# microsoft/GenerativeImage2Text

Hardware: NVIDIA H100
Metric: captions/sec (greedy, max_len=40) GIT_BASE batch64 (higher is better)
Workload: dtype bf16

## Files before the change

### generativeimage2text_b200/csrc/gemm.cuh

```cuda
#pragma once
#include "ptx.cuh"

namespace gitb200 {

struct GemmParams {
  int M, N, K;
  int k_splits;
  int transposed;
  int partial;
  long long split_stride;
  int act;
  int out_bf16;
  const float* bias;
  const float* resid;
  long long ld_resid;
  void* out[3];
  long long ldo;
  long long batch_stride;
  int seg_n;
  int rows_per_batch;
  int row_offset;
  const int* skip;
  unsigned long long* dbg;
  int split3;
  int pdl;
  ChainSync chain;
  const int* lse_target;
};

constexpr int EPI_TRANSPOSED = 1, EPI_BF16 = 2, EPI_RESID = 4, EPI_PARTIAL = 8, EPI_ACT_SHIFT = 4, EPI_SPLIT3 = 64;
constexpr int EPI_LSE = 128;
constexpr int epi_code(bool transposed, bool bf16, bool resid, bool partial, int act) {
  return (transposed ? EPI_TRANSPOSED : 0) | (bf16 ? EPI_BF16 : 0) | (resid ? EPI_RESID : 0) | (partial ? EPI_PARTIAL : 0) |
         (act << EPI_ACT_SHIFT);
}

template <int ACT>
__device__ __forceinline__ float act_ct(float x) {
  return apply_act(x, ACT);
}

template <int BN>
struct GemmCfg {
  static constexpr int BM = 128;
  static constexpr int BK = 64;
  static constexpr int A_BYTES = BM * BK * 2;
  static constexpr int B_BYTES = BN * BK * 2;
  static constexpr int STAGE_BYTES = A_BYTES + B_BYTES;
  static constexpr int MMA_WGS = 2;
  static constexpr int THREADS = 128 * (1 + MMA_WGS);
  static constexpr int WG_STAGING_BYTES = 4 * 32 * 128;
  static constexpr int STAGING_BYTES = MMA_WGS * WG_STAGING_BYTES;
  static constexpr int BAR_BYTES = 256;
  static constexpr int SMEM_LIMIT = 227 * 1024;
  static constexpr int STAGES_RAW = (SMEM_LIMIT - 1024 - BAR_BYTES - STAGING_BYTES) / STAGE_BYTES;
  static constexpr int STAGES = STAGES_RAW > 8 ? 8 : STAGES_RAW;
  static constexpr int SMEM_BYTES = STAGES * STAGE_BYTES + STAGING_BYTES + 1024 + BAR_BYTES;
  static constexpr int PRODUCER_REGS = 40, MMA_REGS = 232;
  static_assert(BN % 64 == 0 && BN >= 64 && BN <= 256, "BN");
  static_assert(B_BYTES % 1024 == 0, "B tile must keep 1024B alignment for SWIZZLE_128B");
  static_assert(2 * STAGES * 8 <= BAR_BYTES, "barrier area");
  static_assert(STAGES >= 3, "pipeline depth");
};

__device__ __forceinline__ uint32_t epi_row_offsets(const GemmParams& p, int row0, int rsub, bool store_ok, long long (&ooff)[8]) {
  uint32_t okmask = 0;
  int bq = (row0 + rsub) / p.rows_per_batch;
  int sq = (row0 + rsub) - bq * p.rows_per_batch;
#pragma unroll
  for (int it = 0; it < 8; ++it) {
    if (row0 + it * 4 + rsub < p.M && store_ok) okmask |= 1u << it;
    ooff[it] = (static_cast<long long>(bq) * p.batch_stride + sq + p.row_offset) * p.ldo;
    sq += 4;
    while (sq >= p.rows_per_batch) { sq -= p.rows_per_batch; ++bq; }
  }
  return okmask;
}

template <int EPI>
__device__ __forceinline__ void epi_store_normal(const GemmParams& p, const uint8_t* stg, int lane, int n0,
                                                 int row0, const long long (&ooff)[8], uint32_t okmask) {
  constexpr bool kBf16 = (EPI & EPI_BF16) != 0;
  constexpr bool kResid = (EPI & EPI_RESID) != 0;
  constexpr int kAct = (EPI >> EPI_ACT_SHIFT) & 3;
  constexpr bool kSplit3 = (EPI & EPI_SPLIT3) != 0;
  static_assert(!kSplit3 || kBf16, "split3 is a bf16 output format");
  const int c4 = lane & 7;
  const int rsub = lane >> 3;
  float4 b4 = make_float4(0.f, 0.f, 0.f, 0.f);
  if (p.bias != nullptr) b4 = __ldg(reinterpret_cast<const float4*>(p.bias + n0) + c4);
  int seg = 0;
  if (p.seg_n < p.N) seg = n0 / p.seg_n;
  const int nn = n0 - seg * p.seg_n + c4 * 4;
  float4 v[8];
#pragma unroll
  for (int it = 0; it < 8; ++it) {
    const int rr = it * 4 + rsub;
    v[it] = *reinterpret_cast<const float4*>(stg + rr * 128 + ((c4 ^ (rr & 7)) << 4));
  }
  float4 res[8];
  if (kResid) {
    const float* rbase = p.resid + static_cast<long long>(row0 + rsub) * p.ld_resid + n0 + c4 * 4;
#pragma unroll
    for (int it = 0; it < 8; ++it) {
      res[it] = make_float4(0.f, 0.f, 0.f, 0.f);
      if (okmask & (1u << it)) res[it] = *reinterpret_cast<const float4*>(rbase + static_cast<long long>(it) * 4 * p.ld_resid);
    }
  }
  uint8_t* obase = reinterpret_cast<uint8_t*>(p.out[seg]) + static_cast<long long>(nn) * (kBf16 ? 2 : 4);
#pragma unroll
  for (int it = 0; it < 8; ++it) {
    float4 o = v[it];
    o.x += b4.x; o.y += b4.y; o.z += b4.z; o.w += b4.w;
    if (kAct != ACT_NONE) {
      o.x = act_ct<kAct>(o.x); o.y = act_ct<kAct>(o.y); o.z = act_ct<kAct>(o.z); o.w = act_ct<kAct>(o.w);
// ... 81 lines not shown
        }
      } else {
        float* dst = reinterpret_cast<float*>(p.out[0]) + off;
        if (full4 && (p.ldo & 3) == 0) {
          *reinterpret_cast<float4*>(dst) = make_float4(v[0], v[1], v[2], v[3]);
        } else if (full4 && (p.ldo & 1) == 0) {
          *reinterpret_cast<float2*>(dst) = make_float2(v[0], v[1]);
          *reinterpret_cast<float2*>(dst + 2) = make_float2(v[2], v[3]);
        } else {
          for (int e = 0; e < 4; ++e)
            if (f0 + e < p.M) dst[e] = v[e];
        }
      }
    }
  }
}

__device__ __forceinline__ void epi_lse_accum(const GemmParams& p, const uint8_t* stg, int lane, int n0, const int (&tgt)[8],
                                              float (&m)[8], float (&se)[8], float (&sx)[8], float (&xt)[8]) {
  const int c4 = lane & 7;
  const int rsub = lane >> 3;
  const int col0 = n0 + c4 * 4;
  float b[4];
  bool ok[4];
#pragma unroll
  for (int e = 0; e < 4; ++e) {
    ok[e] = col0 + e < p.N;
    b[e] = ok[e] ? __ldg(p.bias + col0 + e) : 0.f;
  }
#pragma unroll
  for (int it = 0; it < 8; ++it) {
    const int rr = it * 4 + rsub;
    const float4 v = *reinterpret_cast<const float4*>(stg + rr * 128 + ((c4 ^ (rr & 7)) << 4));
    const float x[4] = {v.x + b[0], v.y + b[1], v.z + b[2], v.w + b[3]};
    float cm = -INFINITY;
#pragma unroll
    for (int e = 0; e < 4; ++e) if (ok[e]) cm = fmaxf(cm, x[e]);
    const float nm = fmaxf(m[it], cm);
    if (nm == -INFINITY) continue;
    float acc = (m[it] == -INFINITY) ? 0.f : se[it] * __expf(m[it] - nm);
#pragma unroll
    for (int e = 0; e < 4; ++e) {
      if (ok[e]) {
        acc += __expf(x[e] - nm);
        sx[it] += x[e];
        if (tgt[it] == col0 + e) xt[it] = x[e];
      }
    }
    se[it] = acc;
    m[it] = nm;
  }
}

template <int BN, int EPI>
__global__ void __launch_bounds__(GemmCfg<BN>::THREADS, 1)
gemm_bf16_wgmma(const __grid_constant__ CUtensorMap tmA, const __grid_constant__ CUtensorMap tmB,
                const GemmParams p) {
  using C = GemmCfg<BN>;
  constexpr bool kTransposed = (EPI & EPI_TRANSPOSED) != 0;
  constexpr bool kLse = (EPI & EPI_LSE) != 0;
  static_assert(!kLse || EPI == EPI_LSE, "the statistics epilogue takes no other option");
  if (p.pdl) griddep_launch_early();
  if (p.pdl) tl_mark(100000 + 1000 + static_cast<int>(gridDim.x));
  if ((!p.pdl || p.chain.counters != nullptr) && p.skip != nullptr && *p.skip != 0) return;
  extern __shared__ __align__(1024) uint8_t smem_raw[];
  uint8_t* smem = smem_raw + ((1024u - (smem_u32(smem_raw) & 1023u)) & 1023u);
  uint8_t* sA = smem;
  uint8_t* sB = smem + C::STAGES * C::A_BYTES;
  uint8_t* sStage = smem + C::STAGES * C::STAGE_BYTES;
  uint64_t* full = reinterpret_cast<uint64_t*>(sStage + C::STAGING_BYTES);
  uint64_t* empty = full + C::STAGES;

  const int wg = threadIdx.x >> 7;
  const int warp = (threadIdx.x >> 5) & 3;
  const int lane = threadIdx.x & 31;

  if (threadIdx.x == 0) {
    tma_prefetch_desc(&tmA);
    tma_prefetch_desc(&tmB);
    for (int s = 0; s < C::STAGES; ++s) {
      mbar_init(&full[s], 1);
      mbar_init(&empty[s], C::MMA_WGS);
    }
    mbar_fence_init();
  }
  __syncthreads();

  const int m_tiles = (p.M + C::BM - 1) / C::BM;
  const int n_tiles = (p.N + BN - 1) / BN;
  const int kb_total = (p.K + C::BK - 1) / C::BK;
  const int kb_per = (kb_total + p.k_splits - 1) / p.k_splits;
  const int mn_tiles = m_tiles * n_tiles;
  const int num_tiles = mn_tiles * p.k_splits;

  const bool chained = p.chain.counters != nullptr;
  int npre = 0;
  if (kTransposed && p.pdl && static_cast<int>(blockIdx.x) < num_tiles) {
    const int split = static_cast<int>(blockIdx.x) / mn_tiles;
    const int kb0 = split * kb_per;
    npre = min(C::STAGES, min(kb_total, kb0 + kb_per) - kb0);
    if (threadIdx.x == 0) {
      const int m_blk = (static_cast<int>(blockIdx.x) - split * mn_tiles) / n_tiles;
      for (int i = 0; i < npre; ++i) {
        mbar_arrive_expect_tx(&full[i], C::STAGE_BYTES);
        tma_load_2d(sA + i * C::A_BYTES, &tmA, &full[i], (kb0 + i) * C::BK, m_blk * C::BM);
      }
    }
  }
  if (chained) chain_wait(p.chain);
  else if (p.pdl) griddep_wait();
  if (p.pdl) tl_mark(1000 + static_cast<int>(gridDim.x));

  if (wg == 0) {
    setmaxnreg_dec<C::PRODUCER_REGS>();
    if (threadIdx.x == 0) {
      int stage = 0;
      uint32_t phase = 0;
      for (int tile = blockIdx.x; tile < num_tiles; tile += gridDim.x) {
        const int split = tile / mn_tiles;
        const int rem = tile - split * mn_tiles;
        const int m_blk = rem / n_tiles;
        const int n_blk = rem - m_blk * n_tiles;
        const int kb0 = split * kb_per;
        const int kb1 = min(kb_total, kb0 + kb_per);
        for (int kb = kb0; kb < kb1; ++kb) {
          if (npre > 0) {
            --npre;
            tma_load_2d(sB + stage * C::B_BYTES, &tmB, &full[stage], kb * C::BK, n_blk * BN);
          } else {
            mbar_wait(&empty[stage], phase ^ 1);
            mbar_arrive_expect_tx(&full[stage], C::STAGE_BYTES);
            tma_load_2d(sA + stage * C::A_BYTES, &tmA, &full[stage], kb * C::BK, m_blk * C::BM);
            tma_load_2d(sB + stage * C::B_BYTES, &tmB, &full[stage], kb * C::BK, n_blk * BN);
          }
          if (++stage == C::STAGES) {
            stage = 0;
            phase ^= 1;
          }
        }
      }
    }
  } else {
    setmaxnreg_inc<C::MMA_REGS>();
    const int mw = wg - 1;
    const bool store_ok = !(p.pdl && !chained && p.skip != nullptr && *p.skip != 0);
    uint8_t* stg_wg = sStage + mw * C::WG_STAGING_BYTES;
    uint8_t* stg = stg_wg + warp * (32 * 128);
    const int rsub = lane >> 3;
    float acc[BN / 2];
    int stage = 0;
    uint32_t phase = 0;
    for (int tile = blockIdx.x; tile < num_tiles; tile += gridDim.x) {
      const int split = tile / mn_tiles;
      const int rem = tile - split * mn_tiles;
      const int m_blk = rem / n_tiles;
      const int n_blk = rem - m_blk * n_tiles;
      const int kb0 = split * kb_per;
      const int kb1 = min(kb_total, kb0 + kb_per);
      int prev = -1;
      for (int kb = kb0; kb < kb1; ++kb) {
        mbar_wait(&full[stage], phase);
        if (p.pdl && tile == static_cast<int>(blockIdx.x) && kb == kb0 && threadIdx.x == 128) tl_mark_one(300000 + 1000 + static_cast<int>(gridDim.x));
        const uint32_t a_base = smem_u32(sA + stage * C::A_BYTES + mw * (64 * 128));
        const uint32_t b_base = smem_u32(sB + stage * C::B_BYTES);
        wgmma_fence();
#pragma unroll
        for (int k = 0; k < C::BK / 16; ++k)
          Wgmma<BN>::mma(acc, wgmma_desc_sw128(a_base + k * 32), wgmma_desc_sw128(b_base + k * 32), (kb > kb0 || k > 0) ? 1u : 0u);
        wgmma_commit();
        if (prev >= 0) {
          wgmma_wait<1>();
          if ((threadIdx.x & 127) == 0) mbar_arrive(&empty[prev]);
        }
        prev = stage;
        if (++stage == C::STAGES) {
          stage = 0;
          phase ^= 1;
        }
      }
      wgmma_wait<0>();
      if ((threadIdx.x & 127) == 0) mbar_arrive(&empty[prev]);
      if (p.pdl && tile == static_cast<int>(blockIdx.x) && threadIdx.x == 128) tl_mark_one(400000 + 1000 + static_cast<int>(gridDim.x));

      const int row0 = m_blk * C::BM + mw * 64 + (warp & 1) * 32;
      long long ooff[8];
      uint32_t okmask = 0;
      if (!kTransposed && !kLse) okmask = epi_row_offsets(p, row0, rsub, store_ok, ooff);
      float lm[8], lse_s[8], lsx[8], lxt[8];
      int ltg[8];
      if constexpr (kLse) {
#pragma unroll
        for (int it = 0; it < 8; ++it) {
          const int row = row0 + it * 4 + rsub;
          ltg[it] = row < p.M ? p.lse_target[row] : -1;
          lm[it] = -INFINITY; lse_s[it] = 0.f; lsx[it] = 0.f; lxt[it] = 0.f;
        }
      }
#pragma unroll
      for (int cc = 0; cc < BN / 64; ++cc) {
        if (n_blk * BN + cc * 64 >= p.N) break;
#pragma unroll
        for (int j8 = 0; j8 < 8; ++j8) {
#pragma unroll
          for (int hh = 0; hh < 2; ++hh) {
            const int r64 = warp * 16 + (lane >> 2) + 8 * hh;
            const int c64 = j8 * 8 + 2 * (lane & 3);
            const int r = r64 & 31, c = c64 & 31;
            uint8_t* blk = stg_wg + ((c64 >> 5) * 2 + (r64 >> 5)) * (32 * 128);
            const float v0 = acc[4 * (cc * 8 + j8) + 2 * hh], v1 = acc[4 * (cc * 8 + j8) + 2 * hh + 1];
            if (!kTransposed) {
              *reinterpret_cast<float2*>(blk + r * 128 + (((c >> 2) ^ (r & 7)) << 4) + (c & 3) * 4) = make_float2(v0, v1);
            } else {
              *reinterpret_cast<float*>(blk + c * 128 + (((r >> 2) ^ (c & 7)) << 4) + (r & 3) * 4) = v0;
              *reinterpret_cast<float*>(blk + (c + 1) * 128 + (((r >> 2) ^ ((c + 1) & 7)) << 4) + (r & 3) * 4) = v1;
            }
          }
        }
        named_bar_sync(1 + mw, 128);
        const int n0 = n_blk * BN + cc * 64 + (warp >> 1) * 32;
        if constexpr (kLse) {
          epi_lse_accum(p, stg, lane, n0, ltg, lm, lse_s, lsx, lxt);
        } else if (!kTransposed) {
          if (n0 < p.N) epi_store_normal<EPI>(p, stg, lane, n0, row0, ooff, okmask);
        } else {
          epi_store_transposed<EPI>(p, stg, lane, n0, row0, split, store_ok);
        }
        named_bar_sync(1 + mw, 128);
      }
      if constexpr (kLse) {
#pragma unroll
        for (int it = 0; it < 8; ++it) {
#pragma unroll
          for (int o = 1; o < 8; o <<= 1) {
            const float m_o = __shfl_xor_sync(0xffffffffu, lm[it], o);
            const float s_o = __shfl_xor_sync(0xffffffffu, lse_s[it], o);
            const float nm = fmaxf(lm[it], m_o);
            const float sa = (lm[it] == -INFINITY) ? 0.f : lse_s[it] * __expf(lm[it] - nm);
            const float sb = (m_o == -INFINITY) ? 0.f : s_o * __expf(m_o - nm);
            lse_s[it] = sa + sb;
            lm[it] = nm;
            lsx[it] += __shfl_xor_sync(0xffffffffu, lsx[it], o);
            lxt[it] += __shfl_xor_sync(0xffffffffu, lxt[it], o);
          }
          const int row = row0 + it * 4 + rsub;
          if ((lane & 7) == 0 && row < p.M)
            reinterpret_cast<float4*>(p.out[0])[static_cast<long long>(row) * p.ldo + 2 * n_blk + (warp >> 1)] =
                make_float4(lm[it], lse_s[it], lsx[it], lxt[it]);
        }
      }
    }
  }

  __syncthreads();
  if (p.pdl) tl_mark(200000 + 1000 + static_cast<int>(gridDim.x));
  if (chained && threadIdx.x == 0) chain_signal_thread0(p.chain);
}

}
```

### generativeimage2text_b200/csrc/gitb200.cu

```cuda
#include <cuda.h>
#include <cuda_bf16.h>
#include <cuda_runtime.h>

#include <algorithm>
#include <cmath>
#include <cstdarg>
#include <cstdio>
#include <cstring>
#include <map>
#include <mutex>
#include <set>
#include <string>
#include <utility>
#include <vector>

#include "../../include/gitb200.h"
#include "attention.cuh"
#include "constrained.cuh"
#include "decode_mega.cuh"
#include "gemm.cuh"
#include "preproc.cuh"
#include "ptx.cuh"
#include "rowops.cuh"
#include "search.cuh"
// ... 1 lines not shown
using namespace gitb200;
typedef __nv_bfloat16 bf16;

#define GITB200_ABI_VERSION 10

static thread_local std::string g_create_error;

struct DevBuf {
  void* p = nullptr;
  size_t cap = 0;
  bool owned = true;
  cudaError_t ensure(size_t bytes) {
    if (bytes <= cap) return cudaSuccess;
    if (!owned) return cudaErrorInvalidValue;
    if (p) cudaFree(p);
    p = nullptr;
    cap = 0;
    cudaError_t e = cudaMalloc(&p, bytes);
    if (e == cudaSuccess) cap = bytes;
    return e;
  }
  void release() {
    if (p && owned) cudaFree(p);
    p = nullptr;
    cap = 0;
    owned = true;
  }
  void borrow(const DevBuf& o) {
    release();
    p = o.p;
    cap = o.cap;
    owned = false;
  }
  template <typename T>
  T* as() const { return reinterpret_cast<T*>(p); }
};

struct EncLayer {
  DevBuf wqkv, bqkv, wo, bo, ln1g, ln1b, ln2g, ln2b, w1, b1, w2, b2;
};
struct DecLayer {
  DevBuf wqkv, bqkv, wo, bo, lnag, lnab, w1, b1, w2, b2, lnog, lnob;
  DevBuf m_wqkv, m_wo, m_w1, m_w2;
};

typedef CUresult (*EncodeTiledFn)(CUtensorMap*, CUtensorMapDataType, cuuint32_t, void*, const cuuint64_t*,
                                  const cuuint64_t*, const cuuint32_t*, const cuuint32_t*, CUtensorMapInterleave,
                                  CUtensorMapSwizzle, CUtensorMapL2promotion, CUtensorMapFloatOOBfill);

struct TmapKey {
  const void* ptr;
  long long rows, cols, ld;
  int box_rows;
  bool operator<(const TmapKey& o) const {
    if (ptr != o.ptr) return ptr < o.ptr;
    if (rows != o.rows) return rows < o.rows;
    if (cols != o.cols) return cols < o.cols;
    if (ld != o.ld) return ld < o.ld;
    return box_rows < o.box_rows;
  }
};

struct DecAttnGeom {
  int chunk_rows, box_rows;
  size_t smem;
  int grid;
};

struct gitb200_engine {
  gitb200_config cfg;
  int device = 0;
  int num_sms = 132;
  std::string err;
  int64_t launches = 0;
  bool use_graph = true;
  bool use_pdl = true;
  bool use_mega = true;
  bool mega_ready = false;
  int debug_layers = -1;
  bool parity = false;
  int ks() const { return parity ? 3 : 1; }
  size_t kvb() const { return parity ? 4 : 2; }
  const gitb200_engine* weights_from = nullptr;

  int g = 0, L = 0, Kpatch = 0, Kp = 0, d = 0, D = 0, F = 0, V = 0;
  int in_h = 0, in_w = 0, gh = 0, gw = 0, Lc = 0;
  std::vector<int> rg_next_hw;
  bool cur_ragged = false;
  std::vector<int> cur_lens;
  DevBuf rg_tab, rg_lens;

  DevBuf w_patch, cls, pos_emb, lnpre_g, lnpre_b, lnpost_g, lnpost_b;
  std::vector<EncLayer> enc;
  DevBuf w_vp, b_vp, lnvp_g, lnvp_b, words_f32, words_bf16, positions, lnemb_g, lnemb_b, out_bias, temb;
  DevBuf m_lm;
  std::vector<DecLayer> dec;
  std::set<std::string> seen;
  bool finalized = false;

  DevBuf x, h, qkv, ctx, u, feats, feats_f32, pos_interp;
  DevBuf pt, pxd, phd, pq, pctx, pu;
  DevBuf img_kv, txt_kv, src_row[2];
  size_t txt_kv_eb = 0;
  DevBuf xd_t, hd_t, qkv_t, ctx_t, t_t, u_t, logits;
  DevBuf y_t, qb_t, mega_bar;
  DevBuf state, next_token, logprob_sum, tokens_i64, stage_img, stage_tok, stage_lp, prefix_dev;
  DevBuf beam_ws;
// ... 45 lines not shown
  va_list ap;
  va_start(ap, fmt);
  vsnprintf(buf, sizeof(buf), fmt, ap);
  va_end(ap);
  if (h) h->err = buf; else g_create_error = buf;
  return 1;
}

#define CK(call)                                                                                     \
  do {                                                                                               \
    cudaError_t e_ = (call);                                                                         \
    if (e_ != cudaSuccess) return fail(h, "%s failed: %s (%s:%d)", #call, cudaGetErrorString(e_), __FILE__, __LINE__); \
  } while (0)
#define CKL(h_, what)                                                                                \
  do {                                                                                               \
    cudaError_t e_ = cudaGetLastError();                                                             \
    if (e_ != cudaSuccess) return fail(h_, "launch %s failed: %s", what, cudaGetErrorString(e_));    \
    (h_)->launches++;                                                                                \
  } while (0)
#define TRY(expr)                 \
  do {                            \
    int rc_ = (expr);             \
    if (rc_ != 0) return rc_;     \
  } while (0)

template <typename... KArgs, typename... Args>
static cudaError_t launch_k(bool pdl, void (*kern)(KArgs...), dim3 grid, dim3 block, size_t smem, cudaStream_t st,
                            Args&&... args) {
  cudaLaunchConfig_t cfg{};
  cfg.gridDim = grid;
  cfg.blockDim = block;
  cfg.dynamicSmemBytes = smem;
  cfg.stream = st;
  cudaLaunchAttribute attr[1];
  attr[0].id = cudaLaunchAttributeProgrammaticStreamSerialization;
  attr[0].val.programmaticStreamSerializationAllowed = 1;
  cfg.attrs = attr;
  cfg.numAttrs = pdl ? 1 : 0;
  return cudaLaunchKernelEx(&cfg, kern, std::forward<Args>(args)...);
}

static int load_encode_fn(gitb200_engine* h) {
  if (h->encode_tiled) return 0;
  void* fn = nullptr;
  cudaDriverEntryPointQueryResult qres;
  cudaError_t e = cudaGetDriverEntryPoint("cuTensorMapEncodeTiled", &fn, cudaEnableDefault, &qres);
  if (e != cudaSuccess || qres != cudaDriverEntryPointSuccess || fn == nullptr)
    return fail(h, "cuTensorMapEncodeTiled not available from the driver: %s", cudaGetErrorString(e));
  h->encode_tiled = reinterpret_cast<EncodeTiledFn>(fn);
  return 0;
}

static int get_tmap(gitb200_engine* h, const void* ptr, long long rows, long long cols, long long ld, int box_rows,
                    CUtensorMap* out, bool swizzle = true) {
  TmapKey key{ptr, rows, cols, ld, swizzle ? box_rows : -box_rows};
  auto it = h->tmaps.find(key);
  if (it != h->tmaps.end()) {
    *out = it->second;
    return 0;
  }
  TRY(load_encode_fn(h));
  if ((reinterpret_cast<uintptr_t>(ptr) & 15) != 0 || (ld * 2) % 16 != 0)
    return fail(h, "TMA operand must be 16-byte aligned with a 16-byte multiple row pitch (ptr=%p ld=%lld)", ptr, ld);
  CUtensorMap m;
  cuuint64_t dims[2] = {static_cast<cuuint64_t>(cols), static_cast<cuuint64_t>(rows)};
  cuuint64_t strides[1] = {static_cast<cuuint64_t>(ld) * 2};
  cuuint32_t box[2] = {64u, static_cast<cuuint32_t>(box_rows)};
  cuuint32_t estr[2] = {1u, 1u};
  CUresult r = h->encode_tiled(&m, CU_TENSOR_MAP_DATA_TYPE_BFLOAT16, 2, const_cast<void*>(ptr), dims, strides, box, estr,
                               CU_TENSOR_MAP_INTERLEAVE_NONE, swizzle ? CU_TENSOR_MAP_SWIZZLE_128B : CU_TENSOR_MAP_SWIZZLE_NONE,
                               CU_TENSOR_MAP_L2_PROMOTION_L2_256B, CU_TENSOR_MAP_FLOAT_OOB_FILL_NONE);
  if (r != CUDA_SUCCESS) return fail(h, "cuTensorMapEncodeTiled failed with CUresult %d (rows=%lld cols=%lld ld=%lld box=%d)",
                                     static_cast<int>(r), rows, cols, ld, box_rows);
  if (h->tmaps.size() > 4096) h->tmaps.clear();
  h->tmaps[key] = m;
  *out = m;
  return 0;
}

struct GemmCall {
  const bf16* A = nullptr;
  long long lda = 0;
  const bf16* B = nullptr;
  long long ldb = 0;
  GemmParams p{};
  int bn = 0;
};

template <int BN, int EPI>
static int launch_gemm_inst(gitb200_engine* h, const GemmCall& c, cudaStream_t st) {
  using C = GemmCfg<BN>;
  static bool attr_set[64] = {false};
  if (!attr_set[h->device & 63]) {
    CK(cudaFuncSetAttribute(gemm_bf16_wgmma<BN, EPI>, cudaFuncAttributeMaxDynamicSharedMemorySize, C::SMEM_BYTES));
    attr_set[h->device & 63] = true;
  }
  CUtensorMap ta, tb;
  TRY(get_tmap(h, c.A, c.p.M, c.p.K, c.lda, 128, &ta));
  TRY(get_tmap(h, c.B, c.p.N, c.p.K, c.ldb, BN, &tb));
  const int m_tiles = (c.p.M + 127) / 128;
  const int n_tiles = (c.p.N + BN - 1) / BN;
  const int tiles = m_tiles * n_tiles * c.p.k_splits;
  const int grid = tiles < h->num_sms ? tiles : h->num_sms;
  h->last_gemm_grid = grid;
  CK(launch_k(c.p.pdl != 0, gemm_bf16_wgmma<BN, EPI>, dim3(grid), dim3(C::THREADS), C::SMEM_BYTES, st, ta, tb, c.p));
  CKL(h, "gemm_bf16_wgmma");
  return 0;
}

template <int BN>
static int launch_gemm_bn(gitb200_engine* h, const GemmCall& c, cudaStream_t st) {
  const GemmParams& p = c.p;
  if constexpr (BN == 256) {
    if (p.lse_target != nullptr) return launch_gemm_inst<BN, EPI_LSE>(h, c, st);
  }
  if (p.lse_target != nullptr) return fail(h, "gemm: the LM-head statistics epilogue runs with 256-column tiles only");
  const int code = epi_code(p.transposed != 0, p.out_bf16 != 0, p.resid != nullptr, p.partial != 0, p.act) | (p.split3 ? EPI_SPLIT3 : 0);
  if constexpr (BN == 256) {
    switch (code) {
      case epi_code(false, true, false, false, ACT_QUICKGELU_EXACT) | EPI_SPLIT3: return launch_gemm_inst<BN, epi_code(false, true, false, false, ACT_QUICKGELU_EXACT) | EPI_SPLIT3>(h, c, st);
      case epi_code(false, true, false, false, ACT_GELU_ERF) | EPI_SPLIT3: return launch_gemm_inst<BN, epi_code(false, true, false, false, ACT_GELU_ERF) | EPI_SPLIT3>(h, c, st);
      default: break;
    }
  }
  if constexpr (BN == 64 || BN == 128 || BN == 256) {
    if (code == (epi_code(true, true, false, false, ACT_GELU_ERF) | EPI_SPLIT3))
      return launch_gemm_inst<BN, epi_code(true, true, false, false, ACT_GELU_ERF) | EPI_SPLIT3>(h, c, st);
  }
  if constexpr (BN == 192 || BN == 256 || BN == 128) {
    switch (code) {
      case epi_code(false, true, false, false, ACT_NONE): return launch_gemm_inst<BN, epi_code(false, true, false, false, ACT_NONE)>(h, c, st);
      case epi_code(false, false, true, false, ACT_NONE): return launch_gemm_inst<BN, epi_code(false, false, true, false, ACT_NONE)>(h, c, st);
      case epi_code(false, false, false, false, ACT_NONE): return launch_gemm_inst<BN, epi_code(false, false, false, false, ACT_NONE)>(h, c, st);
      case epi_code(false, true, false, false, ACT_QUICKGELU): return launch_gemm_inst<BN, epi_code(false, true, false, false, ACT_QUICKGELU)>(h, c, st);
      case epi_code(false, true, false, false, ACT_GELU_ERF): return launch_gemm_inst<BN, epi_code(false, true, false, false, ACT_GELU_ERF)>(h, c, st);
      default: break;
    }
  }
  if constexpr (BN == 64 || BN == 128 || BN == 256) {
    switch (code) {
      case epi_code(true, false, false, true, ACT_NONE): return launch_gemm_inst<BN, epi_code(true, false, false, true, ACT_NONE)>(h, c, st);
      case epi_code(true, false, false, false, ACT_NONE): return launch_gemm_inst<BN, epi_code(true, false, false, false, ACT_NONE)>(h, c, st);
      case epi_code(true, true, false, false, ACT_GELU_ERF): return launch_gemm_inst<BN, epi_code(true, true, false, false, ACT_GELU_ERF)>(h, c, st);
      default: break;
    }
  }
  return fail(h, "gemm: epilogue combination not instantiated (transposed=%d bf16=%d resid=%d partial=%d act=%d bn=%d)",
              p.transposed, p.out_bf16, p.resid != nullptr, p.partial, p.act, BN);
}

static int pick_bn(const gitb200_engine* h, int M, int N, bool transposed) {
  if (transposed) return N <= 64 ? 64 : (N <= 128 ? 128 : 256);
  (void)h; (void)M;
  if (N % 256 == 0 && N >= 1024) return 256;
  if (N % 192 == 0) return 192;
  if (N % 256 == 0) return 256;
  if (N % 128 == 0) return 128;
  return N > 192 ? 256 : (N > 128 ? 192 : 128);
// ... 807 lines not shown
  h->cur_M = frames * L;
  h->cur_ragged = rg;
  return 0;
}

constexpr int kQkvSplits = 3, kOutProjSplits = 6, kFc2Splits = 8, kMaxProjSplits = 8;

static char* img_kv_ptr(gitb200_engine* h, int layer, int kv, long long elem_off = 0) {
  const long long per = static_cast<long long>(h->cur_B) * h->cur_M * h->D;
  return h->img_kv.as<char>() + ((static_cast<long long>(layer) * 2 + kv) * per + elem_off) * h->kvb();
}
static char* txt_kv_ptr(gitb200_engine* h, int layer, int kv, long long elem_off = 0) {
  const long long per = static_cast<long long>(h->cur_rows) * h->T_alloc * h->D;
  return h->txt_kv.as<char>() + ((static_cast<long long>(layer) * 2 + kv) * per + elem_off) * h->kvb();
}

static int decoder_buffers(gitb200_engine* h, long long text_rows) {
  const int D = h->D, F = h->F, nl = h->cfg.dec_layers;
  const long long img_rows = static_cast<long long>(h->cur_B) * h->cur_M;
  const long long rows = std::max(img_rows, text_rows);
  const int ks = h->ks();
  const long long kvb = static_cast<long long>(h->kvb());
  CK(h->pt.ensure(rows * D * 4));
  CK(h->pxd.ensure(rows * D * 4));
  CK(h->phd.ensure(rows * D * 2 * ks));
  CK(h->pq.ensure(rows * D * kvb));
  CK(h->pctx.ensure(rows * D * 2 * ks));
  CK(h->pu.ensure(rows * F * 2 * ks));
  CK(h->img_kv.ensure(static_cast<long long>(nl) * 2 * img_rows * D * kvb));
  return 0;
}

template <typename Attend>
static int decoder_layers(gitb200_engine* h, int rows, char* kv, bool kv_per_layer, bool last_qkv_only, Attend&& attend,
                          cudaStream_t st) {
  const int D = h->D, F = h->F, nl = h->cfg.dec_layers;
  const long long kv_bytes = static_cast<long long>(rows) * D * h->kvb();
  float* t = h->pt.as<float>();
  float* xd = h->pxd.as<float>();
  bf16* hd = h->phd.as<bf16>();
  bf16* ctx = h->pctx.as<bf16>();
  bf16* u = h->pu.as<bf16>();
  auto ln = [&](const DevBuf& g, const DevBuf& b) {
    return launch_ln(h, ln_operand(h, t, g.as<float>(), b.as<float>(), 1e-12f, xd, hd, rows), D, st);
  };
  for (int j = 0; j < nl; ++j) {
    DecLayer& l = h->dec[j];
    char* k = kv + (kv_per_layer ? 2 * j * kv_bytes : 0);
    char* v = k + kv_bytes;
    GemmCall c = gemm_rows(h, RowOut::QKV, hd, l.wqkv.as<bf16>(), rows, 3 * D, D, l.bqkv.as<float>(), ACT_NONE, nullptr, h->pq.p);
    c.p.seg_n = D;
    c.p.out[1] = k; c.p.out[2] = v;
    c.p.ldo = D;
    TRY(launch_gemm(h, c, st));
    if (last_qkv_only && j + 1 == nl) break;
    TRY(attend(j, h->pq.p, k, v, ctx));
    TRY(launch_gemm(h, gemm_rows(h, RowOut::F32, ctx, l.wo.as<bf16>(), rows, D, D, l.bo.as<float>(), ACT_NONE, xd, t), st));
    TRY(ln(l.lnag, l.lnab));
    TRY(launch_gemm(h, gemm_rows(h, RowOut::OPERAND, hd, l.w1.as<bf16>(), rows, F, D, l.b1.as<float>(), ACT_GELU_ERF, nullptr, u), st));
    TRY(launch_gemm(h, gemm_rows(h, RowOut::F32, u, l.w2.as<bf16>(), rows, D, F, l.b2.as<float>(), ACT_NONE, xd, t), st));
    TRY(ln(l.lnog, l.lnob));
  }
  return 0;
}

static int image_rows(gitb200_engine* h, float* vproj_out, cudaStream_t st) {
  const int D = h->D, d = h->d, M = h->cur_M, B = h->cur_B;
  const int rows = B * M;
  float* t = h->pt.as<float>();
  float* xd = h->pxd.as<float>();
  TRY(launch_gemm(h, gemm_rows(h, RowOut::F32, h->feats.as<bf16>(), h->w_vp.as<bf16>(), rows, D, d, h->b_vp.as<float>(), ACT_NONE, nullptr, t), st));
  TRY(launch_ln(h, ln_operand(h, t, h->lnvp_g.as<float>(), h->lnvp_b.as<float>(), 1e-5f, xd, h->phd.as<bf16>(), rows), D, st));
  if (vproj_out) CK(cudaMemcpyAsync(vproj_out, xd, static_cast<size_t>(rows) * D * 4, cudaMemcpyDeviceToDevice, st));
  SelfAttn a{};
  a.B = B; a.S = M; a.H = h->cfg.dec_heads;
  a.q_rs = a.kv_rs = D; a.q_bs = a.kv_bs = static_cast<long long>(M) * D;
  a.o_rs = D * h->ks(); a.o_bs = static_cast<long long>(M) * a.o_rs;
  a.seq_lens = h->cur_ragged ? h->rg_lens.as<int>() : nullptr;
  auto self_attention = [&](int, const void* q, const void* k, const void* v, bf16* ctx) {
    a.q = q; a.k = k; a.v = v; a.out = ctx;
    return launch_self_attention(h, a, h->parity, st);
  };
  return decoder_layers(h, rows, h->img_kv.as<char>(), true, true, self_attention, st);
}

static int prefill_impl(gitb200_engine* h, int B, int beam, int T_alloc, float* vproj_out, cudaStream_t st) {
  if (B != h->cur_B || h->cur_M <= 0) return fail(h, "prefill: call encode with the same batch first");
  const int D = h->D, F = h->F, nl = h->cfg.dec_layers;
  const int R = B * beam;
  const int ks = h->ks();
  const long long kvb = static_cast<long long>(h->kvb());
  TRY(decoder_buffers(h, 0));
  {
    const void* before = h->txt_kv.p;
    CK(h->txt_kv.ensure(static_cast<long long>(nl) * 2 * R * T_alloc * D * kvb));
    if (h->txt_kv.p != before || h->txt_kv_eb != h->kvb()) CK(cudaMemsetAsync(h->txt_kv.p, 0, h->txt_kv.cap, st));
    h->txt_kv_eb = h->kvb();
  }
  CK(h->src_row[0].ensure(static_cast<size_t>(R) * T_alloc * 4));
  CK(h->src_row[1].ensure(static_cast<size_t>(R) * T_alloc * 4));
  CK(h->xd_t.ensure(static_cast<size_t>(R) * D * 4));
  CK(h->hd_t.ensure(static_cast<size_t>(R) * D * 2 * ks));
  CK(h->qkv_t.ensure(static_cast<size_t>(kQkvSplits) * R * 3 * D * 4));
  CK(h->ctx_t.ensure(static_cast<size_t>(R) * D * 2 * ks));
  CK(h->t_t.ensure(static_cast<size_t>(kMaxProjSplits) * R * D * 4));
  CK(h->u_t.ensure(static_cast<size_t>(R) * F * 2 * ks));
  CK(h->logits.ensure(static_cast<size_t>(R) * h->V * 4));
  CK(h->state.ensure(sizeof(StepState) + 64));
// ... 106 lines not shown
```

### generativeimage2text_b200/csrc/ptx.cuh

```cuda
#pragma once
#include <cuda.h>
#include <cuda_bf16.h>
#include <cuda_runtime.h>
#include <stdint.h>

namespace gitb200 {

__device__ __forceinline__ uint32_t smem_u32(const void* p) {
  return static_cast<uint32_t>(__cvta_generic_to_shared(p));
}
__device__ __forceinline__ int lane_id() { return threadIdx.x & 31; }
__device__ __forceinline__ unsigned long long globaltimer_ns() {
  unsigned long long t;
  asm volatile("mov.u64 %0, %%globaltimer;" : "=l"(t));
  return t;
}

#ifdef GITB200_TIMELINE
__device__ unsigned long long* g_tl_buf = nullptr;
__device__ unsigned int g_tl_count = 0;
constexpr unsigned int kTimelineMax = 8192;
__device__ __forceinline__ void tl_mark_one(int kid) {
  if (g_tl_buf != nullptr && blockIdx.x == 0 && blockIdx.y == 0 && blockIdx.z == 0) {
    const unsigned int i = atomicAdd(&g_tl_count, 1u);
// ... 41 lines not shown
__device__ __forceinline__ void chain_signal(const ChainSync& c) {
  if (c.counters != nullptr) {
    __syncthreads();
    if (threadIdx.x == 0) chain_signal_thread0(c);
  }
}

__device__ __forceinline__ void named_bar_sync(int id, int nthreads) {
  asm volatile("bar.sync %0, %1;" ::"r"(id), "r"(nthreads) : "memory");
}

__device__ __forceinline__ void mbar_init(uint64_t* bar, uint32_t count) {
  asm volatile("mbarrier.init.shared::cta.b64 [%0], %1;" ::"r"(smem_u32(bar)), "r"(count) : "memory");
}
__device__ __forceinline__ void mbar_fence_init() {
  asm volatile("fence.mbarrier_init.release.cluster;" ::: "memory");
}
__device__ __forceinline__ void mbar_arrive_expect_tx(uint64_t* bar, uint32_t bytes) {
  asm volatile("mbarrier.arrive.expect_tx.shared::cta.b64 _, [%0], %1;" ::"r"(smem_u32(bar)), "r"(bytes)
               : "memory");
}
__device__ __forceinline__ void mbar_arrive(uint64_t* bar) {
  asm volatile("mbarrier.arrive.shared::cta.b64 _, [%0];" ::"r"(smem_u32(bar)) : "memory");
}
__device__ __forceinline__ bool mbar_try_wait(uint64_t* bar, uint32_t parity) {
  uint32_t ok;
  asm volatile(
      "{\n"
      ".reg .pred p;\n"
      "mbarrier.try_wait.parity.shared::cta.b64 p, [%1], %2;\n"
      "selp.u32 %0, 1, 0, p;\n"
      "}\n"
      : "=r"(ok)
      : "r"(smem_u32(bar)), "r"(parity)
      : "memory");
  return ok != 0;
}
__device__ __forceinline__ void mbar_wait(uint64_t* bar, uint32_t parity) {
  while (!mbar_try_wait(bar, parity)) {
  }
}

__device__ __forceinline__ void tma_prefetch_desc(const CUtensorMap* m) {
  asm volatile("prefetch.tensormap [%0];" ::"l"(reinterpret_cast<uint64_t>(m)) : "memory");
}
__device__ __forceinline__ void tma_load_2d(void* smem_dst, const CUtensorMap* m, uint64_t* bar, int c_inner,
                                            int c_outer) {
  asm volatile(
      "cp.async.bulk.tensor.2d.shared::cluster.global.mbarrier::complete_tx::bytes [%0], [%1, {%3, %4}], [%2];"
      ::"r"(smem_u32(smem_dst)), "l"(reinterpret_cast<uint64_t>(m)), "r"(smem_u32(bar)), "r"(c_inner),
      "r"(c_outer)
      : "memory");
}

__device__ __forceinline__ void wgmma_fence() { asm volatile("wgmma.fence.sync.aligned;" ::: "memory"); }
__device__ __forceinline__ void wgmma_commit() { asm volatile("wgmma.commit_group.sync.aligned;" ::: "memory"); }
template <int N>
__device__ __forceinline__ void wgmma_wait() {
  asm volatile("wgmma.wait_group.sync.aligned %0;" ::"n"(N) : "memory");
}
template <int R>
__device__ __forceinline__ void setmaxnreg_dec() { asm volatile("setmaxnreg.dec.sync.aligned.u32 %0;" ::"n"(R)); }
template <int R>
__device__ __forceinline__ void setmaxnreg_inc() { asm volatile("setmaxnreg.inc.sync.aligned.u32 %0;" ::"n"(R)); }

__device__ __forceinline__ uint64_t wgmma_desc_sw128(uint32_t smem_addr) {
  uint64_t d = 0;
  d |= static_cast<uint64_t>((smem_addr & 0x3FFFF) >> 4);
  d |= static_cast<uint64_t>(1) << 16;
  d |= static_cast<uint64_t>(1024 >> 4) << 32;
  d |= static_cast<uint64_t>(1) << 62;
  return d;
}

template <int N>
struct Wgmma;
template <>
struct Wgmma<64> {
  static __device__ __forceinline__ void mma(float (&d)[32], uint64_t a_desc, uint64_t b_desc, uint32_t accumulate) {
    asm volatile(
        "{\n"
        ".reg .pred p;\n"
        "setp.ne.b32 p, %34, 0;\n"
        "wgmma.mma_async.sync.aligned.m64n64k16.f32.bf16.bf16 "
        "{%0, %1, %2, %3, %4, %5, %6, %7, %8, %9, %10, %11, %12, %13, %14, %15, %16, %17, %18, %19, %20, %21, %22, %23, %24, %25, %26, %27, %28, %29, %30, %31}, %32, %33, p, 1, 1, 0, 0;\n"
        "}\n"
        : "+f"(d[0]), "+f"(d[1]), "+f"(d[2]), "+f"(d[3]), "+f"(d[4]), "+f"(d[5]), "+f"(d[6]), "+f"(d[7]), "+f"(d[8]), "+f"(d[9]), "+f"(d[10]), "+f"(d[11]), "+f"(d[12]), "+f"(d[13]), "+f"(d[14]), "+f"(d[15]), "+f"(d[16]), "+f"(d[17]), "+f"(d[18]), "+f"(d[19]), "+f"(d[20]), "+f"(d[21]), "+f"(d[22]), "+f"(d[23]), "+f"(d[24]), "+f"(d[25]), "+f"(d[26]), "+f"(d[27]), "+f"(d[28]), "+f"(d[29]), "+f"(d[30]), "+f"(d[31])
        : "l"(a_desc), "l"(b_desc), "r"(accumulate));
  }
};
template <>
struct Wgmma<128> {
  static __device__ __forceinline__ void mma(float (&d)[64], uint64_t a_desc, uint64_t b_desc, uint32_t accumulate) {
    asm volatile(
        "{\n"
        ".reg .pred p;\n"
        "setp.ne.b32 p, %66, 0;\n"
        "wgmma.mma_async.sync.aligned.m64n128k16.f32.bf16.bf16 "
        "{%0, %1, %2, %3, %4, %5, %6, %7, %8, %9, %10, %11, %12, %13, %14, %15, %16, %17, %18, %19, %20, %21, %22, %23, %24, %25, %26, %27, %28, %29, %30, %31, %32, %33, %34, %35, %36, %37, %38, %39, %40, %41, %42, %43, %44, %45, %46, %47, %48, %49, %50, %51, %52, %53, %54, %55, %56, %57, %58, %59, %60, %61, %62, %63}, %64, %65, p, 1, 1, 0, 0;\n"
        "}\n"
        : "+f"(d[0]), "+f"(d[1]), "+f"(d[2]), "+f"(d[3]), "+f"(d[4]), "+f"(d[5]), "+f"(d[6]), "+f"(d[7]), "+f"(d[8]), "+f"(d[9]), "+f"(d[10]), "+f"(d[11]), "+f"(d[12]), "+f"(d[13]), "+f"(d[14]), "+f"(d[15]), "+f"(d[16]), "+f"(d[17]), "+f"(d[18]), "+f"(d[19]), "+f"(d[20]), "+f"(d[21]), "+f"(d[22]), "+f"(d[23]), "+f"(d[24]), "+f"(d[25]), "+f"(d[26]), "+f"(d[27]), "+f"(d[28]), "+f"(d[29]), "+f"(d[30]), "+f"(d[31]), "+f"(d[32]), "+f"(d[33]), "+f"(d[34]), "+f"(d[35]), "+f"(d[36]), "+f"(d[37]), "+f"(d[38]), "+f"(d[39]), "+f"(d[40]), "+f"(d[41]), "+f"(d[42]), "+f"(d[43]), "+f"(d[44]), "+f"(d[45]), "+f"(d[46]), "+f"(d[47]), "+f"(d[48]), "+f"(d[49]), "+f"(d[50]), "+f"(d[51]), "+f"(d[52]), "+f"(d[53]), "+f"(d[54]), "+f"(d[55]), "+f"(d[56]), "+f"(d[57]), "+f"(d[58]), "+f"(d[59]), "+f"(d[60]), "+f"(d[61]), "+f"(d[62]), "+f"(d[63])
        : "l"(a_desc), "l"(b_desc), "r"(accumulate));
  }
};
template <>
struct Wgmma<192> {
// ... 127 lines not shown
```

Before: 3115.

## Use TMA bulk stores and prefetched residual loads in the GEMM epilogue

```diff
diff --git a/generativeimage2text_b200/csrc/gemm.cuh b/generativeimage2text_b200/csrc/gemm.cuh
--- a/generativeimage2text_b200/csrc/gemm.cuh
+++ b/generativeimage2text_b200/csrc/gemm.cuh
@@ -26,6 +26,12 @@
   int pdl;
   ChainSync chain;
   const int* lse_target;
+  int tma_epi;
+};
+
+struct EpiMaps {
+  CUtensorMap out[3];
+  CUtensorMap resid;
 };
 
 constexpr int EPI_TRANSPOSED = 1, EPI_BF16 = 2, EPI_RESID = 4, EPI_PARTIAL = 8, EPI_ACT_SHIFT = 4, EPI_SPLIT3 = 64;
@@ -49,7 +55,9 @@
   static constexpr int STAGE_BYTES = A_BYTES + B_BYTES;
   static constexpr int MMA_WGS = 2;
   static constexpr int THREADS = 128 * (1 + MMA_WGS);
-  static constexpr int WG_STAGING_BYTES = 4 * 32 * 128;
+  static constexpr int EPI_BUF_BYTES = 64 * 128;
+  static constexpr int EPI_BUFS = BN == 192 ? 4 : 2;
+  static constexpr int WG_STAGING_BYTES = EPI_BUFS * EPI_BUF_BYTES;
   static constexpr int STAGING_BYTES = MMA_WGS * WG_STAGING_BYTES;
   static constexpr int BAR_BYTES = 256;
   static constexpr int SMEM_LIMIT = 227 * 1024;
@@ -59,8 +67,9 @@
   static constexpr int PRODUCER_REGS = 40, MMA_REGS = 232;
   static_assert(BN % 64 == 0 && BN >= 64 && BN <= 256, "BN");
   static_assert(B_BYTES % 1024 == 0, "B tile must keep 1024B alignment for SWIZZLE_128B");
-  static_assert(2 * STAGES * 8 <= BAR_BYTES, "barrier area");
+  static_assert((2 * STAGES + MMA_WGS * EPI_BUFS) * 8 <= BAR_BYTES, "barrier area");
   static_assert(STAGES >= 3, "pipeline depth");
+  static_assert(BN != 192 || STAGES == 4, "the extra staging of BN = 192 must not cost a pipeline stage");
 };
 
 __device__ __forceinline__ uint32_t epi_row_offsets(const GemmParams& p, int row0, int rsub, bool store_ok, long long (&ooff)[8]) {
@@ -248,13 +257,106 @@
   }
 }
 
+template <int BN>
+__device__ __forceinline__ void epi_resid_prefetch(const GemmParams& p, const EpiMaps& em, uint8_t* stg_wg, uint64_t* rfull,
+                                                   int n0, int grow, uint32_t eseq) {
+  using C = GemmCfg<BN>;
+  bulk_wait_read<0>();
+#pragma unroll
+  for (int j = 0; j < C::EPI_BUFS && j < BN / 32; ++j) {
+    if (n0 + j * 32 >= p.N) break;
+    const int b = (eseq + j) % C::EPI_BUFS;
+    mbar_arrive_expect_tx(&rfull[b], C::EPI_BUF_BYTES);
+    tma_load_2d(stg_wg + b * C::EPI_BUF_BYTES, &em.resid, &rfull[b], n0 + j * 32, grow);
+  }
+}
+
+template <int BN, int EPI>
+__device__ __forceinline__ void epi_tma_tile(const GemmParams& p, const EpiMaps& em, const float (&acc)[BN / 2],
+                                             uint8_t* stg_wg, uint64_t* rfull, int n_blk, int grow, int mw, bool leader,
+                                             bool store_ok, uint32_t& eseq, uint32_t& rphase) {
+  using C = GemmCfg<BN>;
+  constexpr bool kBf16 = (EPI & EPI_BF16) != 0;
+  constexpr bool kResid = (EPI & EPI_RESID) != 0;
+  constexpr int kAct = (EPI >> EPI_ACT_SHIFT) & 3;
+  constexpr int W = kBf16 ? 64 : 32;
+  constexpr int NB = C::EPI_BUFS;
+  static_assert(!kResid || !kBf16, "the residual is added to fp32 output only");
+  const int warp = (threadIdx.x >> 5) & 3;
+  const int lane = threadIdx.x & 31;
+  const int nseg = p.N / p.seg_n;
+#pragma unroll
+  for (int ch = 0; ch < BN / W; ++ch) {
+    const int n0 = n_blk * BN + ch * W;
+    if (n0 >= p.N) break;
+    const int b = eseq % NB;
+    uint8_t* buf = stg_wg + b * C::EPI_BUF_BYTES;
+    if (kResid) {
+      mbar_wait(&rfull[b], (rphase >> b) & 1u);
+      rphase ^= 1u << b;
+    }
+#pragma unroll
+    for (int j8 = 0; j8 < W / 8; ++j8) {
+      const int c = j8 * 8 + 2 * (lane & 3);
+      float2 bv = make_float2(0.f, 0.f);
+      if (p.bias != nullptr) bv = __ldg(reinterpret_cast<const float2*>(p.bias + n0 + c));
+#pragma unroll
+      for (int hh = 0; hh < 2; ++hh) {
+        const int r = warp * 16 + (lane >> 2) + 8 * hh;
+        const int ai = 4 * (ch * (W / 8) + j8) + 2 * hh;
+        float o0 = acc[ai] + bv.x, o1 = acc[ai + 1] + bv.y;
+        if (kAct != ACT_NONE) {
+          o0 = act_ct<kAct>(o0);
+          o1 = act_ct<kAct>(o1);
+        }
+        if (kBf16) {
+          *reinterpret_cast<uint32_t*>(buf + r * 128 + (((c >> 3) ^ (r & 7)) << 4) + (c & 7) * 2) = pack_bf16(o0, o1);
+        } else {
+          float2* dst = reinterpret_cast<float2*>(buf + r * 128 + (((c >> 2) ^ (r & 7)) << 4) + (c & 3) * 4);
+          if (kResid) {
+            const float2 rv = *dst;
+            o0 = rv.x + o0;
+            o1 = rv.y + o1;
+          }
+          *dst = make_float2(o0, o1);
+        }
+      }
+    }
+    fence_proxy_async_smem();
+    if (leader) {
+      if (kResid) {
+        bulk_wait_read<0>();
+        const int na = n0 + (NB - 1) * W;
+        if (ch >= 1 && ch + NB - 1 < BN / W && na < p.N) {
+          const int ba = (eseq + NB - 1) % NB;
+          mbar_arrive_expect_tx(&rfull[ba], C::EPI_BUF_BYTES);
+          tma_load_2d(stg_wg + ba * C::EPI_BUF_BYTES, &em.resid, &rfull[ba], na, grow);
+        }
+      } else {
+        bulk_wait_read<NB - 2>();
+      }
+    }
+    named_bar_sync(1 + mw, 128);
+    if (leader && store_ok) {
+      const int seg = n0 / p.seg_n;
+      const int col = n0 - seg * p.seg_n;
+      tma_store_2d(&em.out[seg], buf, col, grow);
+      if (col + W > p.seg_n && seg + 1 < nseg) tma_store_2d(&em.out[seg + 1], buf, col - p.seg_n, grow);
+      bulk_commit();
+    }
+    ++eseq;
+  }
+}
+
 template <int BN, int EPI>
 __global__ void __launch_bounds__(GemmCfg<BN>::THREADS, 1)
 gemm_bf16_wgmma(const __grid_constant__ CUtensorMap tmA, const __grid_constant__ CUtensorMap tmB,
-                const GemmParams p) {
+                const __grid_constant__ EpiMaps em, const GemmParams p) {
   using C = GemmCfg<BN>;
   constexpr bool kTransposed = (EPI & EPI_TRANSPOSED) != 0;
   constexpr bool kLse = (EPI & EPI_LSE) != 0;
+  constexpr bool kTmaEpi = !kTransposed && !kLse && (EPI & EPI_SPLIT3) == 0;
+  constexpr bool kResid = (EPI & EPI_RESID) != 0;
   static_assert(!kLse || EPI == EPI_LSE, "the statistics epilogue takes no other option");
   if (p.pdl) griddep_launch_early();
   if (p.pdl) tl_mark(100000 + 1000 + static_cast<int>(gridDim.x));
@@ -266,6 +368,7 @@
   uint8_t* sStage = smem + C::STAGES * C::STAGE_BYTES;
   uint64_t* full = reinterpret_cast<uint64_t*>(sStage + C::STAGING_BYTES);
   uint64_t* empty = full + C::STAGES;
+  uint64_t* rfull = empty + C::STAGES;
 
   const int wg = threadIdx.x >> 7;
   const int warp = (threadIdx.x >> 5) & 3;
@@ -278,6 +381,7 @@
       mbar_init(&full[s], 1);
       mbar_init(&empty[s], C::MMA_WGS);
     }
+    for (int b = 0; b < C::MMA_WGS * C::EPI_BUFS; ++b) mbar_init(&rfull[b], 1);
     mbar_fence_init();
   }
   __syncthreads();
@@ -343,6 +447,8 @@
     uint8_t* stg_wg = sStage + mw * C::WG_STAGING_BYTES;
     uint8_t* stg = stg_wg + warp * (32 * 128);
     const int rsub = lane >> 3;
+    const bool leader = (threadIdx.x & 127) == 0;
+    uint32_t eseq = 0, rphase = 0;
     float acc[BN / 2];
     int stage = 0;
     uint32_t phase = 0;
@@ -353,6 +459,7 @@
       const int n_blk = rem - m_blk * n_tiles;
       const int kb0 = split * kb_per;
       const int kb1 = min(kb_total, kb0 + kb_per);
+      const int grow = m_blk * C::BM + mw * 64;
       int prev = -1;
       for (int kb = kb0; kb < kb1; ++kb) {
         mbar_wait(&full[stage], phase);
@@ -364,6 +471,10 @@
         for (int k = 0; k < C::BK / 16; ++k)
           Wgmma<BN>::mma(acc, wgmma_desc_sw128(a_base + k * 32), wgmma_desc_sw128(b_base + k * 32), (kb > kb0 || k > 0) ? 1u : 0u);
         wgmma_commit();
+        if constexpr (kTmaEpi && kResid) {
+          if (kb == kb0 && p.tma_epi && leader && grow < p.M)
+            epi_resid_prefetch<BN>(p, em, stg_wg, rfull + mw * C::EPI_BUFS, n_blk * BN, grow, eseq);
+        }
         if (prev >= 0) {
           wgmma_wait<1>();
           if ((threadIdx.x & 127) == 0) mbar_arrive(&empty[prev]);
@@ -377,6 +488,13 @@
       wgmma_wait<0>();
       if ((threadIdx.x & 127) == 0) mbar_arrive(&empty[prev]);
       if (p.pdl && tile == static_cast<int>(blockIdx.x) && threadIdx.x == 128) tl_mark_one(400000 + 1000 + static_cast<int>(gridDim.x));
+      if constexpr (kTmaEpi) {
+        if (p.tma_epi) {
+          if (grow < p.M)
+            epi_tma_tile<BN, EPI>(p, em, acc, stg_wg, rfull + mw * C::EPI_BUFS, n_blk, grow, mw, leader, store_ok, eseq, rphase);
+          continue;
+        }
+      }
 
       const int row0 = m_blk * C::BM + mw * 64 + (warp & 1) * 32;
       long long ooff[8];
@@ -445,6 +563,9 @@
         }
       }
     }
+    if constexpr (kTmaEpi) {
+      if (leader) bulk_wait_all();
+    }
   }
 
   __syncthreads();
diff --git a/generativeimage2text_b200/csrc/gitb200.cu b/generativeimage2text_b200/csrc/gitb200.cu
--- a/generativeimage2text_b200/csrc/gitb200.cu
+++ b/generativeimage2text_b200/csrc/gitb200.cu
@@ -77,7 +77,9 @@
   const void* ptr;
   long long rows, cols, ld;
   int box_rows;
+  int elem_bytes;
   bool operator<(const TmapKey& o) const {
+    if (elem_bytes != o.elem_bytes) return elem_bytes < o.elem_bytes;
     if (ptr != o.ptr) return ptr < o.ptr;
     if (rows != o.rows) return rows < o.rows;
     if (cols != o.cols) return cols < o.cols;
@@ -229,22 +231,23 @@
 }
 
 static int get_tmap(gitb200_engine* h, const void* ptr, long long rows, long long cols, long long ld, int box_rows,
-                    CUtensorMap* out, bool swizzle = true) {
-  TmapKey key{ptr, rows, cols, ld, swizzle ? box_rows : -box_rows};
+                    CUtensorMap* out, bool swizzle = true, int elem_bytes = 2) {
+  TmapKey key{ptr, rows, cols, ld, swizzle ? box_rows : -box_rows, elem_bytes};
   auto it = h->tmaps.find(key);
   if (it != h->tmaps.end()) {
     *out = it->second;
     return 0;
   }
   TRY(load_encode_fn(h));
-  if ((reinterpret_cast<uintptr_t>(ptr) & 15) != 0 || (ld * 2) % 16 != 0)
+  if ((reinterpret_cast<uintptr_t>(ptr) & 15) != 0 || (ld * elem_bytes) % 16 != 0)
     return fail(h, "TMA operand must be 16-byte aligned with a 16-byte multiple row pitch (ptr=%p ld=%lld)", ptr, ld);
   CUtensorMap m;
   cuuint64_t dims[2] = {static_cast<cuuint64_t>(cols), static_cast<cuuint64_t>(rows)};
-  cuuint64_t strides[1] = {static_cast<cuuint64_t>(ld) * 2};
-  cuuint32_t box[2] = {64u, static_cast<cuuint32_t>(box_rows)};
+  cuuint64_t strides[1] = {static_cast<cuuint64_t>(ld) * elem_bytes};
+  cuuint32_t box[2] = {128u / elem_bytes, static_cast<cuuint32_t>(box_rows)};
   cuuint32_t estr[2] = {1u, 1u};
-  CUresult r = h->encode_tiled(&m, CU_TENSOR_MAP_DATA_TYPE_BFLOAT16, 2, const_cast<void*>(ptr), dims, strides, box, estr,
+  CUresult r = h->encode_tiled(&m, elem_bytes == 4 ? CU_TENSOR_MAP_DATA_TYPE_FLOAT32 : CU_TENSOR_MAP_DATA_TYPE_BFLOAT16, 2,
+                               const_cast<void*>(ptr), dims, strides, box, estr,
                                CU_TENSOR_MAP_INTERLEAVE_NONE, swizzle ? CU_TENSOR_MAP_SWIZZLE_128B : CU_TENSOR_MAP_SWIZZLE_NONE,
                                CU_TENSOR_MAP_L2_PROMOTION_L2_256B, CU_TENSOR_MAP_FLOAT_OOB_FILL_NONE);
   if (r != CUDA_SUCCESS) return fail(h, "cuTensorMapEncodeTiled failed with CUresult %d (rows=%lld cols=%lld ld=%lld box=%d)",
@@ -275,12 +278,25 @@
   CUtensorMap ta, tb;
   TRY(get_tmap(h, c.A, c.p.M, c.p.K, c.lda, 128, &ta));
   TRY(get_tmap(h, c.B, c.p.N, c.p.K, c.ldb, BN, &tb));
-  const int m_tiles = (c.p.M + 127) / 128;
-  const int n_tiles = (c.p.N + BN - 1) / BN;
-  const int tiles = m_tiles * n_tiles * c.p.k_splits;
+  GemmParams p = c.p;
+  EpiMaps em{};
+  const int eb = p.out_bf16 ? 2 : 4;
+  const int nseg = p.N / p.seg_n;
+  bool tma_epi = (EPI & (EPI_TRANSPOSED | EPI_LSE | EPI_SPLIT3)) == 0 && p.rows_per_batch == p.batch_stride &&
+                 p.row_offset == 0 && (p.ldo * eb) % 16 == 0 &&
+                 (p.resid == nullptr || ((p.ld_resid * 4) % 16 == 0 && (reinterpret_cast<uintptr_t>(p.resid) & 15) == 0));
+  for (int s = 0; s < nseg; ++s) tma_epi = tma_epi && (reinterpret_cast<uintptr_t>(p.out[s]) & 15) == 0;
+  if (tma_epi) {
+    for (int s = 0; s < nseg; ++s) TRY(get_tmap(h, p.out[s], p.M, p.seg_n, p.ldo, 64, &em.out[s], true, eb));
+    if (p.resid != nullptr) TRY(get_tmap(h, p.resid, p.M, p.N, p.ld_resid, 64, &em.resid, true, 4));
+    p.tma_epi = 1;
+  }
+  const int m_tiles = (p.M + 127) / 128;
+  const int n_tiles = (p.N + BN - 1) / BN;
+  const int tiles = m_tiles * n_tiles * p.k_splits;
   const int grid = tiles < h->num_sms ? tiles : h->num_sms;
   h->last_gemm_grid = grid;
-  CK(launch_k(c.p.pdl != 0, gemm_bf16_wgmma<BN, EPI>, dim3(grid), dim3(C::THREADS), C::SMEM_BYTES, st, ta, tb, c.p));
+  CK(launch_k(p.pdl != 0, gemm_bf16_wgmma<BN, EPI>, dim3(grid), dim3(C::THREADS), C::SMEM_BYTES, st, ta, tb, em, p));
   CKL(h, "gemm_bf16_wgmma");
   return 0;
 }
@@ -1194,8 +1210,15 @@
     c.p.seg_n = D;
     c.p.out[1] = k; c.p.out[2] = v;
     c.p.ldo = D;
+    const bool kv_only = last_qkv_only && j + 1 == nl;
+    if (kv_only) {
+      c.B += static_cast<long long>(D) * c.ldb;
+      c.p.bias += D;
+      c.p.N = 2 * D;
+      c.p.out[0] = k; c.p.out[1] = v; c.p.out[2] = nullptr;
+    }
     TRY(launch_gemm(h, c, st));
-    if (last_qkv_only && j + 1 == nl) break;
+    if (kv_only) break;
     TRY(attend(j, h->pq.p, k, v, ctx));
     TRY(launch_gemm(h, gemm_rows(h, RowOut::F32, ctx, l.wo.as<bf16>(), rows, D, D, l.bo.as<float>(), ACT_NONE, xd, t), st));
     TRY(ln(l.lnag, l.lnab));
diff --git a/generativeimage2text_b200/csrc/ptx.cuh b/generativeimage2text_b200/csrc/ptx.cuh
--- a/generativeimage2text_b200/csrc/ptx.cuh
+++ b/generativeimage2text_b200/csrc/ptx.cuh
@@ -117,6 +117,17 @@
       "r"(c_outer)
       : "memory");
 }
+
+__device__ __forceinline__ void tma_store_2d(const CUtensorMap* m, const void* smem_src, int c_inner, int c_outer) {
+  asm volatile("cp.async.bulk.tensor.2d.global.shared::cta.bulk_group [%0, {%2, %3}], [%1];"
+               ::"l"(reinterpret_cast<uint64_t>(m)), "r"(smem_u32(smem_src)), "r"(c_inner), "r"(c_outer)
+               : "memory");
+}
+__device__ __forceinline__ void bulk_commit() { asm volatile("cp.async.bulk.commit_group;" ::: "memory"); }
+template <int N>
+__device__ __forceinline__ void bulk_wait_read() { asm volatile("cp.async.bulk.wait_group.read %0;" ::"n"(N) : "memory"); }
+__device__ __forceinline__ void bulk_wait_all() { asm volatile("cp.async.bulk.wait_group 0;" ::: "memory"); }
+__device__ __forceinline__ void fence_proxy_async_smem() { asm volatile("fence.proxy.async.shared::cta;" ::: "memory"); }
 
 __device__ __forceinline__ void wgmma_fence() { asm volatile("wgmma.fence.sync.aligned;" ::: "memory"); }
 __device__ __forceinline__ void wgmma_commit() { asm volatile("wgmma.commit_group.sync.aligned;" ::: "memory"); }
```

New measurement: 3162 (median of 6 runs). Within noise of the previous version (+1.5%).
